# gabraham/flashpca

Measured on AMD Instinct MI355X. Metric: genotype cells/sec (N x P x iters) for k=20 PCA, higher is better.
Workload: dtype i8 (integer genotypes x 7 byte slices of the f64 operand; exact i32 accumulation, f64 recombination; agrees with the f64 kernels to ~3e-15, see fp64_mode); 1 GPU; cfg3: synthetic 500000 samples x 100000 SNPs total, SNP-sharded across GPUs, k=20 (BASELINE configs[2]/[3]); samples=500000, snps_total=100000, snps_per_gpu=100000, k=20, blockvec=16, solver_default_blockvec=16, parallelism=snp-shard x1 + all-reduce(N x b) [single]

## Files before the change

flashpca_amd/_lib.py:

```python
import ctypes as C
import os
import subprocess

HERE = os.path.dirname(os.path.abspath(__file__))
LIB_PATH = os.environ.get("FPCA_LIB") or os.path.join(HERE, "_build", "libfpca.so")
if LIB_PATH == "testhooks":
    LIB_PATH = os.path.join(HERE, "_build", "testhooks", "libfpca.so")
CLI_PATH = os.path.join(HERE, "_build", "flashpca")
HOOKS_LIB_PATH = os.path.join(HERE, "_build", "testhooks", "libfpca.so")
HOOKS_CLI_PATH = os.path.join(HERE, "_build", "testhooks", "flashpca")
CSRC = os.path.join(HERE, "csrc")

STANDARDISE = {"binom": 2, "binom2": 3}
STANDARDISE_DENSE = {"none": 0, "sd": 1, "binom": 2, "binom2": 3, "center": 4}
DIVISOR = {"none": 0, "n1": 1, "p": 2}
UNIQUE_ID_BYTES = 128
SCCA_STATUS = {0: "ok", 1: "maxiter reached", 2: "lambda1 too large", 3: "lambda2 too large"}

ALLREDUCE_FN = C.CFUNCTYPE(C.c_int, C.c_void_p, C.c_void_p, C.c_uint64, C.c_void_p)
COLLECTIVE_FN = C.CFUNCTYPE(C.c_int, C.c_void_p, C.c_void_p, C.c_void_p, C.c_uint64, C.c_void_p)


class PcaOpts(C.Structure):
    _fields_ = [
# ... 120 lines not shown
    "fpca_comm_init_rank": (_I, [_P, _I, _I, _P]),
    "fpca_set_allreduce": (_I, [_P, ALLREDUCE_FN, _P]),
    "fpca_set_collectives": (_I, [_P, COLLECTIVE_FN, COLLECTIVE_FN, _P]),
    "fpca_set_total_snps": (_I, [_P, _U64]),
    "fpca_set_rank": (_I, [_P, _I, _I]),
    "fpca_collective_stats": (_I, [_P, C.POINTER(_U64), C.POINTER(_U64)]),
    "fpca_pca_init_opts": (None, [C.POINTER(PcaOpts), C.c_size_t, C.c_size_t]),
    "fpca_pca_row_ranges": (_I, [_P, C.POINTER(PcaOpts), C.POINTER(_U64), _I]),
    "fpca_pca": (_I, [_P, C.POINTER(PcaOpts), _P, _P, _P, _P, _P, _P, C.POINTER(PcaInfo)]),
    "fpca_check": (_I, [_P, _P, C.c_int64, _P, _I, _I, _P, C.POINTER(_D), C.POINTER(_D)]),
    "fpca_ucca": (_I, [_P, _P, C.c_int64, _I, _I, _P, C.c_int64]),
    "fpca_scca_prepare": (_I, [_P, _P, C.c_int64, _I, _I, _I]),
    "fpca_scca_fit": (_I, [_P, _D, _D, _I, _I, _D, _P, C.c_int64, _P, C.c_int64, _P, C.c_int64, _P, _P, C.c_int64, _P, C.c_int64,
                           C.POINTER(_I), _P, _P, _P, C.POINTER(_I)]),
    "fpca_scca_cv": (_I, [_P, _P, C.c_int64, _I, _P, _I, _P, _I, _P, _I, _I, _I, _I, _I, _D, _P, C.c_int64, C.c_int64, _D, _I, _P, _P, _P, _P, _P, _P,
                          C.POINTER(_D), C.POINTER(_D), C.POINTER(_D), _P, _P]),
    "fpca_bench_apply": (_I, [_P, _I, _I, _I, C.POINTER(BenchResult)]),
    "fpca_profile_begin": (_I, [_P, _I]),
    "fpca_profile_sample_every": (_I, [_P, _I]),
    "fpca_profile_end": (_I, [_P, _I, C.POINTER(BenchResult), C.POINTER(_I)]),
    "fpca_bench_stats": (_I, [_P, _I, C.POINTER(_D), C.POINTER(_D)]),
    "fpca_debug_mfma_probe": (_I, [_P, _P, _P]),
    "fpca_debug_mfma_i8_probe": (_I, [_P, _P, _P]),
    "fpca_debug_mfma_peak": (_I, [_I, _I, _I, C.POINTER(_D)]),
    "fpca_debug_k4": (_I, [_P, _I, _I, _P, _P, _P, _P, _I, _P, _P]),
    "fpca_debug_k4_bench": (_I, [_P, _I, _I, _I, C.POINTER(_D), C.POINTER(_D)]),
    "fpca_debug_k4_fused": (_I, [_P, _I, _I, _P, _P, _P, _P, _P]),
    "fpca_debug_k4_fused_bench": (_I, [_P, _I, _I, _I, C.POINTER(_D)]),
    "fpca_debug_k4_inplace": (_I, [_P, _I, _I, _P, _P, _P, _I, _P, _P]),
    "fpca_debug_fp_plan": (_I, [_P, _I, C.POINTER(_I)]),
    "fpca_debug_poison_partials": (_I, [_P]),
    "fpca_debug_missing_lists": (_I, [_P, _I, _I, _P, _P, _U64, C.POINTER(_U64)]),
    "fpca_debug_gather": (_I, [_I, _I, _P, _P, _U64, _P, _U64, _P, _P, _P, _U64, _U64, _I, _D, _P, C.POINTER(_I)]),
    "fpca_debug_i8_nsc_pad": (_I, [_I, _I, C.POINTER(_I)]),
    "fpca_debug_i8_slices": (_I, [_I, _I, _I, _U64, _U64, _U64, _P, _P, _P, _P, _I, C.POINTER(SlicesOut), C.POINTER(SlicesOut), C.POINTER(_I)]),
    "fpca_debug_i8_instances": (_I, [_P, _I, C.POINTER(_I)]),
    "fpca_debug_gather_blocks": (_I, [_I, _I, _I, _I, _I, _U64, C.POINTER(C.c_uint32), C.POINTER(C.c_uint32), C.POINTER(C.c_uint32)]),
    "fpca_debug_f_sf":(_I, [_D, _U64, _I, C.POINTER(_D), C.POINTER(_D)]),
    "fpca_debug_f_sf_dev": (_I, [_P, _U64, _U64, _I, _P, _P]),
    "fpca_debug_scca_lds": (_I, [_I, C.POINTER(_I), C.POINTER(_I), C.POINTER(_I)]),
    "fpca_debug_fold_stats": (_I, [_P, _P, _I, _P, _I, _P]),
    "fpca_debug_snp_qc_rule": (_I, [_P, _P, _U64, _U64, _D, _D, _P, C.POINTER(_U64)]),
    "fpca_debug_snp_subset_bench": (_I, [_P, _P, _I, C.POINTER(_D), C.POINTER(_D)]),
    "fpca_debug_ld_prune_rule": (_I, [_P, _U64, C.c_uint32, C.c_uint32, _P, _P, _P, _P, C.POINTER(_U64)]),
    "fpca_bench_ld": (_I, [_P, C.c_uint32, _I, _P, C.POINTER(_D)]),
    "fpca_debug_king_rule": (_I, [_P, _P, _U64, _U64, _P, C.POINTER(_U64)]),
# ... 77 lines not shown
```

flashpca_amd/csrc/kernels.hpp:

```cpp
#pragma once
#include <hip/hip_runtime.h>

#include <cstddef>
#include <cstdint>

namespace fpca {
namespace kern {

void repitch(const uint8_t *src, uint64_t np, uint64_t nrec, uint8_t *dst, size_t pitch, hipStream_t stream);
void fix_last_byte(uint8_t *packed, size_t pitch, uint64_t np, int valid_in_last, uint64_t P_g, hipStream_t stream);
void gather_records(const uint8_t *src, size_t pitch, const uint32_t *idx, uint64_t nrec, uint8_t *dst, hipStream_t stream);
void ld_totals(const uint8_t *packed, size_t pitch, uint64_t nrec, uint32_t *tot, hipStream_t stream);
void ld_band(const uint8_t *packed, size_t pitch, const uint32_t *tot, uint32_t npad, uint64_t i0, uint64_t ni, uint64_t jend, uint32_t span,
             double *r2, uint32_t *bits, uint32_t words, double thr, bool force_general, hipStream_t stream);

void bed_stats(const uint8_t *packed, size_t pitch, uint64_t N, uint64_t P_g, int stand_method, double *lut,
               double *mean, double *sd, double *sumsq, uint32_t *nmiss , hipStream_t stream);
void lut_from_meansd(const double *mean, const double *sd, uint64_t P_g, double *lut, hipStream_t stream);

void xt_b(const uint8_t *packed, size_t pitch, const double *lut, const double *B, double *Tpart, uint64_t N_pad,
          uint64_t P_pad, int b, int nsplit, bool fp32, hipStream_t stream);
void x_t(const uint8_t *packed, size_t pitch, const double *lut, const double *T, double *Ypart, uint64_t N_pad,
         uint64_t P_pad, int b, int nsplit, bool fp32, hipStream_t stream);
void reduce_sum(const double *part, double *out, uint64_t count, int nsplit, hipStream_t stream);
// ... 67 lines not shown
   if (!tiled) return (size_t)(r * pitch + q * 16);
   const uint64_t c = q >> 2, kh = (q >> 1) & 1, h = q & 1;
   return (size_t)((r >> 5) * 32 * pitch + c * 2048 + (h * 64 + kh * 32 + (r & 31)) * 16);
}
int gemm_i8_nsc_pad(int S, int b);
size_t gemm_i8_workspace_doubles(uint64_t rows_pad, uint64_t k_pad, int S, int b, bool two);
int gemm_i8_instances(int (*out)[6], int cap);
struct CuFootprint {
   int waves, vgprs, lds_bytes;
};
CuFootprint gemm_i8_footprint(uint64_t rows_pad, int S, int b, bool two, int mode, bool e_only, bool tiled);
void gemm_i8(const uint8_t *packed, size_t pitch, const int8_t *Qg, const int8_t *Qm, const double *wg, const double *wm,
             const long long *colsum_m, const double *mean, const double *sd, double *out, double *ws, uint64_t rows_pad, uint64_t k_pad,
             uint64_t rows_valid, int mode ,
             const double *eplane , int b, int S,
             const SliceOp *next_ops, hipStream_t stream, hipEvent_t *gemm_events = nullptr, hipEvent_t before_combine = nullptr,
             bool e_only = false ,
             bool tiled = false );
void i8_rowscales(const double *mean, const double *sd, uint64_t P_g, uint64_t P_pad, double *inv_sd, double *mu_inv_sd,
                  hipStream_t stream);
void transpose_packed(const uint8_t *in, size_t pitch_in, uint64_t N_pad, uint64_t P_pad, uint8_t *out, size_t pitch_out,
                      hipStream_t stream, bool tiled = false );
void tile_packed(const uint8_t *in, size_t pitch, uint64_t rows, uint8_t *out, hipStream_t stream);
double mfma_i8_peak_tops(int waves_per_simd, int iters, uint32_t fill, hipStream_t stream);
void mfma_i8_probe(const int8_t *A, const int8_t *Bt, int *D, hipStream_t stream);

void gather_packed_rows(const uint8_t *src, size_t pitch, const uint32_t *idx, uint32_t nidx, uint32_t rows_out, uint8_t *dst, hipStream_t stream);
void patch_missing_rows(uint8_t *packed, size_t pitch, const uint32_t *idx, uint32_t nidx, hipStream_t stream);
void scatter_packed_rows(const uint8_t *src, size_t pitch, const uint32_t *idx, uint32_t nidx, uint8_t *packed, hipStream_t stream);
void gather_scaled_rows(const double *V, const double *scale, const uint32_t *idx, uint32_t nidx, uint64_t rows_out, int b, double *dst, hipStream_t stream);
void scatter_rows(const double *src, const uint32_t *idx, uint32_t nidx, int b, double *dst, hipStream_t stream);
void count_missing(const uint8_t *packed, size_t pitch, uint64_t ncols, uint64_t nrec, uint32_t *cnt, hipStream_t stream, bool tiled = false);
void fill_missing(const uint8_t *packed, size_t pitch, uint64_t ncols, uint64_t nrec, const uint32_t *ptr, uint32_t *idx, hipStream_t stream,
                  bool tiled = false);
void sparse_rows_sum(const uint32_t *ptr, const uint32_t *idx, const double *V, const double *rowscale, int b, uint64_t nrec,
                     uint64_t rows_out, double *out, hipStream_t stream, const double *init = nullptr ,
                     bool short_lists = false ,
                     double avg_len = 0 ,
                     unsigned block_limit = 0 );
void sparse_rows_sum_f32(const uint32_t *ptr, const uint32_t *idx, const float *V, const double *colw, int b, uint64_t nrec, uint64_t rows_out,
                         double *out, hipStream_t stream, const double *init = nullptr, bool short_lists = false, double avg_len = 0,
                         unsigned block_limit = 0);
int sparse_rows_sum_variant(int b, bool rowscale, bool short_lists, double avg_len);
unsigned gather_blocks_beside(const CuFootprint &gemm, int gather_vgprs, int ncu);
unsigned sparse_rows_sum_grid(uint64_t rows_out, unsigned block_limit);
unsigned sparse_rows_sum_blocks_beside(const CuFootprint &gemm, int b, bool f32, bool rowscale, bool short_lists, double avg_len);

}
// ... 2 lines not shown
```

flashpca_amd/csrc/kernels_i8.hip:

```cpp
#include <hip/hip_runtime.h>

#include <algorithm>
#include <cmath>
#include <cstdio>
#include <cstdlib>
#include <cstring>
#include <type_traits>
#include <utility>

#include "common.hpp"
#include "dev_scratch.hpp"
#include "kernels.hpp"
#include "launch_check.hpp"

namespace fpca {
namespace kern {

typedef int v4i __attribute__((ext_vector_type(4)));
typedef int v16i __attribute__((ext_vector_type(16)));
typedef double d2 __attribute__((ext_vector_type(2)));
typedef uint32_t u4 __attribute__((ext_vector_type(4)));
typedef uint32_t u2 __attribute__((ext_vector_type(2)));


// ... 520 lines not shown
   const bool idle = C::WAVES == 8 && __builtin_amdgcn_readfirstlane((int)(row0 + (uint64_t)(wr * 32 * MT) >= rows_pad)) != 0;

   v16i acc[MATS][MT][NT];
   v4i acch[MATS][MT][2];
#pragma unroll
   for (int a = 0; a < MATS; a++)
#pragma unroll
      for (int m = 0; m < MT; m++) acch[a][m][0] = acch[a][m][1] = (v4i){0, 0, 0, 0};
#pragma unroll
   for (int a = 0; a < MATS; a++)
#pragma unroll
      for (int m = 0; m < MT; m++)
#pragma unroll
         for (int n = 0; n < NT; n++)
#pragma unroll
            for (int r = 0; r < 16; r++) acc[a][m][n][r] = 0;

   const uint32_t qvoff = (uint32_t)((tid / C::SEGS) * k_pad + (tid % C::SEGS) * 16);
   const uint32_t lds_base = (uint32_t)(size_t)(__attribute__((address_space(3))) unsigned char *)smem;
   const int qdst = (tid / C::SEGS) * LDQ + (tid % C::SEGS) * 16;
   uint32_t pvoff[MT];
#pragma unroll
   for (int m = 0; m < MT; m++)
      pvoff[m] = C::TILED ? (uint32_t)((wr * MT + m) * 32 * pitch + lane * 16)
                          : (uint32_t)((wr * 32 * MT + 32 * m + li) * pitch + kh * (KC / 8));
   const uint8_t *prow = packed + row0 * pitch;
   const uint32_t aQ0 = lds_base + (uint32_t)(wc * 32 * NT + li) * LDQ + kh * (KC / 2);
   const uint32_t aQh0 = lds_base + (uint32_t)(32 * NTF * LDQ + (lane & 15) * C::LDQH) + ((lane >> 5) & 1) * (KC / 2) + ((lane >> 4) & 1) * 16;

   const uint32_t qvoffh = (uint32_t)((tid / 32) * k_pad + (tid % 32) * 8);
   const int qdsth = (tid / 32) * C::LDQH + (tid % 32) * 8;
   u4 qreg[NP];
   u2 qregh[NQ];
   u4 pk[MT][PW], pkn[MT][PW];

   auto issue_q = [&](auto rr, int cc) {
      constexpr int r = decltype(rr)::value, o = r / NP1, r1 = r % NP1;
      const int8_t *sb = ((TWO && o) ? Qm : Qg) + (uint64_t)(col0 + C::RSTEP * r1) * k_pad + (uint64_t)cc * KC;
      if constexpr (C::HALF8 && r1 == NP1 - 1)
         qregh[o] = gload8(sb, qvoffh);
      else
         qreg[r] = gload16<0>(sb, qvoff);
   };
   auto issue_p = [&](u4(&dst)[MT][PW], int cc) {
      const uint8_t *pb = prow + (size_t)cc * (C::TILED ? 2048 : KC / 4);
#pragma unroll
      for (int m = 0; m < MT; m++) {
         dst[m][0] = gload16<0, C::NT_P>(pb, pvoff[m]);
         if constexpr (PW == 2) dst[m][1] = gload16<(C::TILED ? 1024 : 16), C::NT_P>(pb, pvoff[m]);
      }
   };
   auto store_q = [&](auto rr, unsigned char *st, auto behind) {
      constexpr int r = decltype(rr)::value, o = r / NP1, r1 = r % NP1, NB = decltype(behind)::value;
      if constexpr (C::HALF8 && r1 == NP1 - 1) {
         vm_wait<NP - 1 - r + NB>(qregh[o]);
         *reinterpret_cast<u2 *>(st - qdst + qdsth + o * C::QTILE + r1 * C::RSTEP * LDQ) = qregh[o];
      } else {
         vm_wait<NP - 1 - r + NB>(qreg[r]);
         const int hoff = (HALF && r1 == NP1 - 1) ? (tid / C::SEGS) * (C::LDQH - LDQ) : 0;
         *reinterpret_cast<u4 *>(st + o * C::QTILE + r1 * C::RSTEP * LDQ + hoff) = qreg[r];
      }
   };

   constexpr std::integral_constant<int, NPK> after_p{};
   constexpr std::integral_constant<int, 0> after_none{};
   const int c_second = (c_begin + 1 < c_end) ? c_begin + 1 : c_begin;
   if (idle) {
      static_for<NP>([&](auto rr) { issue_q(rr, c_begin); });
      static_for<NP>([&](auto rr) { store_q(rr, smem + qdst, after_none); });
      if constexpr (NBUF == 3) {
         asm volatile("s_waitcnt lgkmcnt(0)" ::: "memory");
         static_for<NP>([&](auto rr) { issue_q(rr, c_second); });
// ... 111 lines not shown
         if constexpr (s == H - 1) issue_p(pkn, cn);
         if constexpr (s >= H) {
            static_for<(s - H + 1) * NP / H - (s - H) * NP / H>([&](auto jj) {
               store_q(std::integral_constant<int, (s - H) * NP / H + decltype(jj)::value>{}, wst, after_p);
            });
         }
         if constexpr (bkey1 != bkey)
            read_b(std::integral_constant<int, ks1>{}, std::integral_constant<int, g1>{}, std::integral_constant<int, (bkey1 & 1)>{}, aQ, aQ2, aQh);
         constexpr bool ahead = NBUF == 3 && last;
         if constexpr (ahead) {
            static_assert(G == 1 && ((NSTEP / MT - 1) & 1) == 1 && ((NSTEP - 1) & AMASK) != 0, "the last micro-step leaves bq[0] and ag[0] free");
#pragma unroll
            for (int mm = 0; mm < MT; mm++)
#pragma unroll
               for (int h = 0; h < PW; h++) {
                  vm_wait<0>(pkn[mm][h]);
                  pk[mm][h] = pkn[mm][h];
               }
            read_b(i0, i0, i0, aQ0 + (uint32_t)bufn * C::STAGE, aQ0 + (uint32_t)bufn * C::STAGE + C::QTILE, aQh0);
         }
         static_for<NG>([&](auto jj) {
            constexpr int j = decltype(jj)::value, n = g * NG + j;
            if constexpr (n < NTF) {
               acc[0][m][n] = __builtin_amdgcn_mfma_i32_32x32x32_i8(ag[akey & AMASK], bq[bkey & 1][0][j], acc[0][m][n], 0, 0, 0);
               if constexpr (MODE == I8_FULL)
                  acc[1][m][n] = __builtin_amdgcn_mfma_i32_32x32x32_i8(am[akey & AMASK], bq[bkey & 1][NQ - 1][j], acc[1][m][n], 0, 0, 0);
            }
            if constexpr (j == 0 && akey1 != akey)
               enz[akey1 & AMASK] = i8_decode<MODE>(pk[m1][ks1 >> 2][ks1 & 3], ag[akey1 & AMASK], am[akey1 & AMASK], tab1);
            if constexpr (j == 0 && ahead) enz[0] = i8_decode<MODE>(pk[0][0][0], ag[0], am[0], tab1);
         });
         if constexpr (HALF && (ks & 1) == 1) {
            v4i t0 = ag[m], t1 = ag[2 + m];
#pragma unroll
            for (int q = 0; q < 4; q++) {
               const auto r = __builtin_amdgcn_permlane16_swap((unsigned)t0[q], (unsigned)t1[q], false, false);
               t0[q] = (int)r[0];
               t1[q] = (int)r[1];
            }
            acch[0][m][0] = __builtin_amdgcn_mfma_i32_16x16x64_i8(t0, bqh, acch[0][m][0], 0, 0, 0);
            acch[0][m][1] = __builtin_amdgcn_mfma_i32_16x16x64_i8(t1, bqh, acch[0][m][1], 0, 0, 0);
            if constexpr (MATS == 2) {
               v4i u0 = am[m], u1 = am[2 + m];
#pragma unroll
               for (int q = 0; q < 4; q++) {
                  const auto r = __builtin_amdgcn_permlane16_swap((unsigned)u0[q], (unsigned)u1[q], false, false);
                  u0[q] = (int)r[0];
                  u1[q] = (int)r[1];
               }
               acch[1][m][0] = __builtin_amdgcn_mfma_i32_16x16x64_i8(u0, TWO ? bqh2 : bqh, acch[1][m][0], 0, 0, 0);
               acch[1][m][1] = __builtin_amdgcn_mfma_i32_16x16x64_i8(u1, TWO ? bqh2 : bqh, acch[1][m][1], 0, 0, 0);
            }
         }
         if constexpr (MODE == I8_SKIP_EMPTY) {
            if (enz[akey & AMASK]) {
               static_for<NG>([&](auto jj) {
                  constexpr int j = decltype(jj)::value, n = g * NG + j;
                  if constexpr (n < NT)
                     acc[1][m][n] = __builtin_amdgcn_mfma_i32_32x32x32_i8(am[akey & AMASK], bq[bkey & 1][NQ - 1][j], acc[1][m][n], 0, 0, 0);
               });
            }
         }
         __builtin_amdgcn_sched_barrier(0);
         if constexpr (bkey1 != bkey) {
            wait_b(std::integral_constant<int, g1>{}, std::integral_constant<int, (bkey1 & 1)>{});
            __builtin_amdgcn_sched_barrier(0);
         }
         if constexpr (ahead) {
            wait_b(i0, i0);
            __builtin_amdgcn_sched_barrier(0);
         }
      });
      if constexpr (NBUF == 3) {
         asm volatile("s_waitcnt lgkmcnt(0)" ::: "memory");
         __builtin_amdgcn_s_barrier();
         asm volatile("" ::: "memory");
         __builtin_amdgcn_sched_barrier(0);
         buf = bufn;
      } else {
#pragma unroll
         for (int m = 0; m < MT; m++)
#pragma unroll
            for (int h = 0; h < PW; h++) {
               vm_wait<0>(pkn[m][h]);
               pk[m][h] = pkn[m][h];
            }
         __syncthreads();
      }
   }

   const int tile0 = (col0 + wc * 32 * NT) / 32;
   double *out = (split == 0 ? part + (((size_t)zblk * rows_pad + row0 + wr * 32 * MT) * 2) * bw
                             : part + (size_t)zb * rows_pad * 2 * bw +
                                  ((((size_t)(split - 1) * zb + zblk) * rowsB + (row0 - rowB0) + wr * 32 * MT) * 2) * bw) +
                 li;
   __syncthreads();
   constexpr int WREG = NT * 4096;
   double *sW = reinterpret_cast<double *>(smem + C::WAVES * WREG);
   constexpr int WCOLS = C::WC * NT * 32;
   for (int t = tid; t < WCOLS; t += C::THREADS) {
      sW[t] = t < C::COLS ? wg[col0 + t] : 0.0;
      sW[WCOLS + t] = t < C::COLS ? wm[col0 + t] : 0.0;
   }
   __syncthreads();
   static_assert(C::LDS_BYTES >= C::WAVES * WREG + 2 * WCOLS * 8, "epilogue LDS layout");
   if (idle) return;
   int *sT = reinterpret_cast<int *>(smem + wave * WREG);
   const double *sWl = sW + wc * 32 * NT + li;
   const int kb = bw / 32;
#pragma unroll
   for (int a = 0; a < MATS; a++)
#pragma unroll
      for (int m = 0; m < MT; m++) {
#pragma unroll
         for (int n = 0; n < NTF; n++) {
            const v16i v = acc[a][m][n];
#pragma unroll
            for (int r = 0; r < 16; r++) sT[(n * 32 + (r & 3) + 8 * (r >> 2) + 4 * kh) * 32 + li] = v[r];
            __builtin_amdgcn_sched_barrier(0);
         }
         if constexpr (HALF) {
#pragma unroll
            for (int t = 0; t < 2; t++)
#pragma unroll
               for (int r = 0; r < 4; r++) {
                  const int row = 16 * t + 4 * (lane >> 4) + r;
                  sT[(NTF * 32 + row) * 32 + (lane & 15)] = acch[a][m][t][r];
                  sT[(NTF * 32 + row) * 32 + 16 + (lane & 15)] = 0;
               }
         }
         __builtin_amdgcn_fence(__ATOMIC_RELEASE, "wavefront");
         __builtin_amdgcn_wave_barrier();
         for (int j = 0; j < 16; j++) {
            const int row = 16 * kh + j;
            for (int k = 0; k < kb; k++) {
               double acc64 = 0.0;
               for (int n = NT - 1 - ((NT - 1 - k) % kb); n >= 0; n -= kb)
                  acc64 += sWl[a * WCOLS + 32 * n] * (double)sT[(n * 32 + row) * 32 + li];
               out[((size_t)(32 * m + row) * 2 + a) * bw + 32 * ((tile0 + k) % kb)] = acc64;
            }
         }
         __builtin_amdgcn_fence(__ATOMIC_ACQUIRE, "wavefront");
         __builtin_amdgcn_wave_barrier();
      }
}

__global__ __launch_bounds__(256) void k_i8_combine(const double *__restrict__ part, int zb, int rows_tile, int nA, int sB, uint64_t rowB0,
                                                     uint64_t rowsB, uint64_t rows_pad, uint64_t rows_valid, int mats,
                                                     const double *__restrict__ eplane ,
                                                     int b, int bw, int S,
                                                     const double *__restrict__ wm, const long long *__restrict__ colsum_m ,
                                                     const double *__restrict__ mean, const double *__restrict__ sd,
                                                     double *__restrict__ out, const double *__restrict__ rs0,
                                                     unsigned long long *__restrict__ bits0, const double *__restrict__ rs1,
                                                     unsigned long long *__restrict__ bits1)
{
   __shared__ double smax[256], sw[9 * 64], sones[64];
   const int c = threadIdx.x % b, r_in = threadIdx.x / b, r_step = 256 / b;
   double m0 = 0.0, m1 = 0.0;
   for (int t = threadIdx.x; t < S * b; t += 256) sw[t] = (mats < 0 || !colsum_m) ? 0.0 : wm[t] * (double)colsum_fold(colsum_m, t);
   __syncthreads();
   if ((int)threadIdx.x < b) {
// ... 445 lines not shown
   if (rows % 256 || pitch % 64) throw Error(-1, "tile_packed: rows in multiples of 256, whole 64-byte chunks per row");
   if (!rows) return;
   hipLaunchKernelGGL(k_tile_packed, dim3((unsigned)(pitch / 64), (unsigned)(rows / 256)), dim3(256), 0, stream, in, pitch, out);
   launch_check();
}

__global__ void k_mfma_i8_probe(const int8_t *A , const int8_t *Bt , int *D)
{
   const int lane = threadIdx.x & 63, li = lane & 31, kh = lane >> 5;
   v4i a = *reinterpret_cast<const v4i *>(A + li * 32 + kh * 16);
   v4i b = *reinterpret_cast<const v4i *>(Bt + li * 32 + kh * 16);
   v16i acc;
   for (int r = 0; r < 16; r++) acc[r] = 0;
   acc = __builtin_amdgcn_mfma_i32_32x32x32_i8(a, b, acc, 0, 0, 0);
   for (int r = 0; r < 16; r++) D[((r & 3) + 8 * (r >> 2) + 4 * kh) * 32 + li] = acc[r];
}

void mfma_i8_probe(const int8_t *A, const int8_t *Bt, int *D, hipStream_t stream)
{
   hipLaunchKernelGGL(k_mfma_i8_probe, dim3(1), dim3(64), 0, stream, A, Bt, D);
   launch_check();
}

__global__ __launch_bounds__(256, 1) void k_mfma_i8_peak(int *out, int iters, uint32_t fill)
{
   const uint32_t l = threadIdx.x * 2654435761u;
   const uint32_t f0 = fill ? (fill ^ l) * 0x9E3779B1u : 0u, f1 = fill ? (f0 >> 3) * 0x85EBCA6Bu : 0u, f2 = fill ? (f1 >> 5) * 0xC2B2AE35u : 0u,
                  f3 = fill ? (f2 >> 7) * 0x27D4EB2Fu : 0u;
   asm volatile(
      "v_mov_b32 v0, 0\n\t"
      "v_mov_b32 v1, 0\n\t"
      "v_mov_b32 v2, 0\n\t"
      "v_mov_b32 v3, 0\n\t"
      "v_mov_b32 v4, 0\n\t"
      "v_mov_b32 v5, 0\n\t"
      "v_mov_b32 v6, 0\n\t"
      "v_mov_b32 v7, 0\n\t"
      "v_mov_b32 v8, 0\n\t"
      "v_mov_b32 v9, 0\n\t"
      "v_mov_b32 v10, 0\n\t"
      "v_mov_b32 v11, 0\n\t"
      "v_mov_b32 v12, 0\n\t"
      "v_mov_b32 v13, 0\n\t"
      "v_mov_b32 v14, 0\n\t"
      "v_mov_b32 v15, 0\n\t"
      "v_mov_b32 v16, 0\n\t"
      "v_mov_b32 v17, 0\n\t"
      "v_mov_b32 v18, 0\n\t"
      "v_mov_b32 v19, 0\n\t"
      "v_mov_b32 v20, 0\n\t"
      "v_mov_b32 v21, 0\n\t"
// ... 83 lines not shown
      "v_mov_b32 v105, 0\n\t"
      "v_mov_b32 v106, 0\n\t"
      "v_mov_b32 v107, 0\n\t"
      "v_mov_b32 v108, 0\n\t"
      "v_mov_b32 v109, 0\n\t"
      "v_mov_b32 v110, 0\n\t"
      "v_mov_b32 v111, 0\n\t"
      "v_mov_b32 v112, 0\n\t"
      "v_mov_b32 v113, 0\n\t"
      "v_mov_b32 v114, 0\n\t"
      "v_mov_b32 v115, 0\n\t"
      "v_mov_b32 v116, 0\n\t"
      "v_mov_b32 v117, 0\n\t"
      "v_mov_b32 v118, 0\n\t"
      "v_mov_b32 v119, 0\n\t"
      "v_mov_b32 v120, 0\n\t"
      "v_mov_b32 v121, 0\n\t"
      "v_mov_b32 v122, 0\n\t"
      "v_mov_b32 v123, 0\n\t"
      "v_mov_b32 v124, 0\n\t"
      "v_mov_b32 v125, 0\n\t"
      "v_mov_b32 v126, 0\n\t"
      "v_mov_b32 v127, 0\n\t"
      ::: "v0", "v1", "v2", "v3", "v4", "v5", "v6", "v7", "v8", "v9", "v10", "v11", "v12", "v13", "v14", "v15", "v16", "v17", "v18", "v19", "v20", "v21", "v22", "v23", "v24", "v25", "v26", "v27", "v28", "v29", "v30", "v31", "v32", "v33", "v34", "v35", "v36", "v37", "v38", "v39", "v40", "v41", "v42", "v43", "v44", "v45", "v46", "v47", "v48", "v49", "v50", "v51", "v52", "v53", "v54", "v55", "v56", "v57", "v58", "v59", "v60", "v61", "v62", "v63", "v64", "v65", "v66", "v67", "v68", "v69", "v70", "v71", "v72", "v73", "v74", "v75", "v76", "v77", "v78", "v79", "v80", "v81", "v82", "v83", "v84", "v85", "v86", "v87", "v88", "v89", "v90", "v91", "v92", "v93", "v94", "v95", "v96", "v97", "v98", "v99", "v100", "v101", "v102", "v103", "v104", "v105", "v106", "v107", "v108", "v109", "v110", "v111", "v112", "v113", "v114", "v115", "v116", "v117", "v118", "v119", "v120", "v121", "v122", "v123", "v124", "v125", "v126", "v127", "v128", "v129", "v130", "v131", "v132", "v133", "v134", "v135", "v136", "v137", "v138", "v139", "v140", "v141", "v142", "v143");
   asm volatile(
      "v_mov_b32 v128, %0\n\t"
      "v_mov_b32 v129, %1\n\t"
      "v_mov_b32 v130, %2\n\t"
      "v_mov_b32 v131, %3\n\t"
      "v_mov_b32 v132, %0\n\t"
      "v_mov_b32 v133, %1\n\t"
      "v_mov_b32 v134, %2\n\t"
      "v_mov_b32 v135, %3\n\t"
      "v_mov_b32 v136, %0\n\t"
      "v_mov_b32 v137, %1\n\t"
      "v_mov_b32 v138, %2\n\t"
      "v_mov_b32 v139, %3\n\t"
      "v_mov_b32 v140, %0\n\t"
      "v_mov_b32 v141, %1\n\t"
      "v_mov_b32 v142, %2\n\t"
      "v_mov_b32 v143, %3\n\t"
      :: "v"(f0), "v"(f1), "v"(f2), "v"(f3) : "v0", "v1", "v2", "v3", "v4", "v5", "v6", "v7", "v8", "v9", "v10", "v11", "v12", "v13", "v14", "v15", "v16", "v17", "v18", "v19", "v20", "v21", "v22", "v23", "v24", "v25", "v26", "v27", "v28", "v29", "v30", "v31", "v32", "v33", "v34", "v35", "v36", "v37", "v38", "v39", "v40", "v41", "v42", "v43", "v44", "v45", "v46", "v47", "v48", "v49", "v50", "v51", "v52", "v53", "v54", "v55", "v56", "v57", "v58", "v59", "v60", "v61", "v62", "v63", "v64", "v65", "v66", "v67", "v68", "v69", "v70", "v71", "v72", "v73", "v74", "v75", "v76", "v77", "v78", "v79", "v80", "v81", "v82", "v83", "v84", "v85", "v86", "v87", "v88", "v89", "v90", "v91", "v92", "v93", "v94", "v95", "v96", "v97", "v98", "v99", "v100", "v101", "v102", "v103", "v104", "v105", "v106", "v107", "v108", "v109", "v110", "v111", "v112", "v113", "v114", "v115", "v116", "v117", "v118", "v119", "v120", "v121", "v122", "v123", "v124", "v125", "v126", "v127", "v128", "v129", "v130", "v131", "v132", "v133", "v134", "v135", "v136", "v137", "v138", "v139", "v140", "v141", "v142", "v143");
   for (int it = 0; it < iters; it++) {
      asm volatile(
         "v_mfma_i32_32x32x32_i8 v[0:15], v[128:131], v[136:139], v[0:15]\n\t"
         "v_mfma_i32_32x32x32_i8 v[16:31], v[132:135], v[136:139], v[16:31]\n\t"
         "v_mfma_i32_32x32x32_i8 v[32:47], v[128:131], v[140:143], v[32:47]\n\t"
         "v_mfma_i32_32x32x32_i8 v[48:63], v[132:135], v[140:143], v[48:63]\n\t"
         "v_mfma_i32_32x32x32_i8 v[64:79], v[128:131], v[136:139], v[64:79]\n\t"
         "v_mfma_i32_32x32x32_i8 v[80:95], v[132:135], v[136:139], v[80:95]\n\t"
         "v_mfma_i32_32x32x32_i8 v[96:111], v[128:131], v[140:143], v[96:111]\n\t"
         "v_mfma_i32_32x32x32_i8 v[112:127], v[132:135], v[140:143], v[112:127]\n\t"
         ::: "v0", "v1", "v2", "v3", "v4", "v5", "v6", "v7", "v8", "v9", "v10", "v11", "v12", "v13", "v14", "v15", "v16", "v17", "v18", "v19", "v20", "v21", "v22", "v23", "v24", "v25", "v26", "v27", "v28", "v29", "v30", "v31", "v32", "v33", "v34", "v35", "v36", "v37", "v38", "v39", "v40", "v41", "v42", "v43", "v44", "v45", "v46", "v47", "v48", "v49", "v50", "v51", "v52", "v53", "v54", "v55", "v56", "v57", "v58", "v59", "v60", "v61", "v62", "v63", "v64", "v65", "v66", "v67", "v68", "v69", "v70", "v71", "v72", "v73", "v74", "v75", "v76", "v77", "v78", "v79", "v80", "v81", "v82", "v83", "v84", "v85", "v86", "v87", "v88", "v89", "v90", "v91", "v92", "v93", "v94", "v95", "v96", "v97", "v98", "v99", "v100", "v101", "v102", "v103", "v104", "v105", "v106", "v107", "v108", "v109", "v110", "v111", "v112", "v113", "v114", "v115", "v116", "v117", "v118", "v119", "v120", "v121", "v122", "v123", "v124", "v125", "v126", "v127", "v128", "v129", "v130", "v131", "v132", "v133", "v134", "v135", "v136", "v137", "v138", "v139", "v140", "v141", "v142", "v143");
   }
   int r;
   asm volatile("s_nop 7\n\ts_nop 7\n\tv_mov_b32 %0, v0" : "=v"(r)::"v0", "v1", "v2", "v3", "v4", "v5", "v6", "v7", "v8", "v9", "v10", "v11", "v12", "v13", "v14", "v15", "v16", "v17", "v18", "v19", "v20", "v21", "v22", "v23", "v24", "v25", "v26", "v27", "v28", "v29", "v30", "v31", "v32", "v33", "v34", "v35", "v36", "v37", "v38", "v39", "v40", "v41", "v42", "v43", "v44", "v45", "v46", "v47", "v48", "v49", "v50", "v51", "v52", "v53", "v54", "v55", "v56", "v57", "v58", "v59", "v60", "v61", "v62", "v63", "v64", "v65", "v66", "v67", "v68", "v69", "v70", "v71", "v72", "v73", "v74", "v75", "v76", "v77", "v78", "v79", "v80", "v81", "v82", "v83", "v84", "v85", "v86", "v87", "v88", "v89", "v90", "v91", "v92", "v93", "v94", "v95", "v96", "v97", "v98", "v99", "v100", "v101", "v102", "v103", "v104", "v105", "v106", "v107", "v108", "v109", "v110", "v111", "v112", "v113", "v114", "v115", "v116", "v117", "v118", "v119", "v120", "v121", "v122", "v123", "v124", "v125", "v126", "v127", "v128", "v129", "v130", "v131", "v132", "v133", "v134", "v135", "v136", "v137", "v138", "v139", "v140", "v141", "v142", "v143");
   if (r == 0x7fffffff) out[threadIdx.x] = r;
}

double mfma_i8_peak_tops(int waves_per_simd, int iters, uint32_t fill, hipStream_t stream)
{
   DevMem<int> d(1024, "fpca_debug_mfma_peak", "the probe's output words");
   const int blocks = 256 * waves_per_simd;
   DevEvent e0("fpca_debug_mfma_peak"), e1("fpca_debug_mfma_peak");
   hipLaunchKernelGGL(k_mfma_i8_peak, dim3(blocks), dim3(256), 0, stream, d.p, iters / 10, fill);
   (void)hipEventRecord(e0, stream);
   hipLaunchKernelGGL(k_mfma_i8_peak, dim3(blocks), dim3(256), 0, stream, d.p, iters, fill);
   (void)hipEventRecord(e1, stream);
   (void)hipEventSynchronize(e1);
   const float ms = elapsed_ms(e0, e1);
   const double ops = (double)blocks * 4  * (double)iters * 8 * 65536.0;
   return ops / (ms * 1e-3) / 1e12;
}

}
}
```

include/fpca_debug.h:

```cpp
#ifndef FPCA_DEBUG_H
#define FPCA_DEBUG_H

#include "fpca.h"

#ifdef __cplusplus
extern "C" {
#endif

typedef struct fpca_bench_result {
   double ms_total;
   double ms_xt;
   double ms_x;
   double ms_allreduce;
   double flops_per_step;
   double packed_bytes_per_step;
   double ms_gemm_xt;
   double ms_gemm_x;
} fpca_bench_result;
int fpca_bench_apply(fpca_ctx *ctx, int b, int steps, int warmup, fpca_bench_result *res);
int fpca_profile_begin(fpca_ctx *ctx, int max_steps);
int fpca_profile_sample_every(fpca_ctx *ctx, int stride);
int fpca_profile_end(fpca_ctx *ctx, int b, fpca_bench_result *res, int *nsteps);
int fpca_bench_stats(fpca_ctx *ctx, int reps, double *ms_per_launch, double *bytes_per_launch);

int fpca_debug_mfma_probe(const double *A, const double *B, double *D);
int fpca_debug_mfma_i8_probe(const int8_t *A, const int8_t *Bt, int32_t *D);
int fpca_debug_mfma_peak(int waves_per_simd, int iters, int pattern, double *tflops);
int fpca_debug_k4(fpca_ctx *ctx, int b, int nq, const double *V, const double *W, double *C_gram, const double *C_in, int use_init,
                  double *Out, double *G_out);
int fpca_debug_k4_fused(fpca_ctx *ctx, int b, int nq, const double *V, const double *W, const double *C_in, double *Out, double *Cg);
int fpca_debug_k4_fused_bench(fpca_ctx *ctx, int b, int nq, int reps, double *ms_fused);
int fpca_debug_k4_inplace(fpca_ctx *ctx, int b, int nq, const double *V, const double *W, const double *C_in, int mode, double *Out,
                          double *G_out);
int fpca_debug_k4_bench(fpca_ctx *ctx, int b, int nq, int reps, double *ms_gram, double *ms_gemm);

int fpca_debug_fp_plan(fpca_ctx *ctx, int b, int out[6]);
int fpca_debug_poison_partials(fpca_ctx *ctx);

int fpca_debug_missing_lists(fpca_ctx *ctx, int b, int by_sample, uint32_t *ptr_out, uint32_t *idx_out, uint64_t idx_cap, uint64_t *nnz);
int fpca_debug_gather(int b, int use_f32, const uint32_t *ptr, const uint32_t *idx, uint64_t nnz, const void *V, uint64_t v_rows,
                      const double *rowscale, const double *colw, const double *init, uint64_t nrec, uint64_t rows_out, int short_lists,
                      double avg_len, double *out, int *variant);

typedef struct fpca_debug_slices_out {
   double *colmax;
   uint64_t *maxbits_own;
   uint64_t *maxbits;
   int8_t *Q;
   int8_t *Qrm;
// ... 42 lines not shown
```

Measured before the change: 80340 billion cells/s.

## Swap MFMA i8 operand order so accumulators hold transposed tiles, vectorise epilogue stores

Exchanges the A and B operands of every i8 MFMA in the gemm kernel so each lane's accumulators hold output columns rather than rows. The epilogue is rewritten to match: LDS staging is transposed, per-lane output pointers change, and results are written as paired double2 stores with two accumulators per loop step. The tiled packed-load offsets are also restructured to share one base offset plus a per-m pointer bump. The likely aim is more contiguous global writes and less per-lane address arithmetic, at the cost of a delicate index remap that must stay exactly consistent with the MFMA output layout. It also adds a debug kernel that checks operand-exchanged MFMA layouts and extends the peak-throughput probe with per-operand fill patterns and a second issue order.

New measurement: 85250 billion cells/s (median of 6 runs). +6.1%, better.

```diff
diff --git a/flashpca_amd/_lib.py b/flashpca_amd/_lib.py
--- a/flashpca_amd/_lib.py
+++ b/flashpca_amd/_lib.py
@@ -166,6 +166,7 @@
     "fpca_bench_stats": (_I, [_P, _I, C.POINTER(_D), C.POINTER(_D)]),
     "fpca_debug_mfma_probe": (_I, [_P, _P, _P]),
     "fpca_debug_mfma_i8_probe": (_I, [_P, _P, _P]),
+    "fpca_debug_mfma_i8_ports": (_I, [_I, _I, _P, _P, _P]),
     "fpca_debug_mfma_peak": (_I, [_I, _I, _I, C.POINTER(_D)]),
     "fpca_debug_k4": (_I, [_P, _I, _I, _P, _P, _P, _P, _I, _P, _P]),
     "fpca_debug_k4_bench": (_I, [_P, _I, _I, _I, C.POINTER(_D), C.POINTER(_D)]),
diff --git a/flashpca_amd/csrc/kernels.hpp b/flashpca_amd/csrc/kernels.hpp
--- a/flashpca_amd/csrc/kernels.hpp
+++ b/flashpca_amd/csrc/kernels.hpp
@@ -113,8 +113,15 @@
 void transpose_packed(const uint8_t *in, size_t pitch_in, uint64_t N_pad, uint64_t P_pad, uint8_t *out, size_t pitch_out,
                       hipStream_t stream, bool tiled = false );
 void tile_packed(const uint8_t *in, size_t pitch, uint64_t rows, uint8_t *out, hipStream_t stream);
-double mfma_i8_peak_tops(int waves_per_simd, int iters, uint32_t fill, hipStream_t stream);
+enum { I8_FILL_ZERO = 0, I8_FILL_RANDOM = 1 , I8_FILL_GENO = 2  };
+struct I8PeakFill {
+   uint32_t seed[4];
+   uint32_t kind[4];
+   int order;
+};
+double mfma_i8_peak_tops(int waves_per_simd, int iters, const I8PeakFill &fill, hipStream_t stream);
 void mfma_i8_probe(const int8_t *A, const int8_t *Bt, int *D, hipStream_t stream);
+void mfma_i8_ports(int shape , bool exchanged, const int8_t *A, const int8_t *Bt, int *D, hipStream_t stream);
 
 void gather_packed_rows(const uint8_t *src, size_t pitch, const uint32_t *idx, uint32_t nidx, uint32_t rows_out, uint8_t *dst, hipStream_t stream);
 void patch_missing_rows(uint8_t *packed, size_t pitch, const uint32_t *idx, uint32_t nidx, hipStream_t stream);
diff --git a/flashpca_amd/csrc/kernels_i8.hip b/flashpca_amd/csrc/kernels_i8.hip
--- a/flashpca_amd/csrc/kernels_i8.hip
+++ b/flashpca_amd/csrc/kernels_i8.hip
@@ -566,7 +566,7 @@
    uint32_t pvoff[MT];
 #pragma unroll
    for (int m = 0; m < MT; m++)
-      pvoff[m] = C::TILED ? (uint32_t)((wr * MT + m) * 32 * pitch + lane * 16)
+      pvoff[m] = C::TILED ? (uint32_t)(wr * MT * 32 * pitch + lane * 16)
                           : (uint32_t)((wr * 32 * MT + 32 * m + li) * pitch + kh * (KC / 8));
    const uint8_t *prow = packed + row0 * pitch;
    const uint32_t aQ0 = lds_base + (uint32_t)(wc * 32 * NT + li) * LDQ + kh * (KC / 2);
@@ -590,8 +590,9 @@
       const uint8_t *pb = prow + (size_t)cc * (C::TILED ? 2048 : KC / 4);
 #pragma unroll
       for (int m = 0; m < MT; m++) {
-         dst[m][0] = gload16<0, C::NT_P>(pb, pvoff[m]);
-         if constexpr (PW == 2) dst[m][1] = gload16<(C::TILED ? 1024 : 16), C::NT_P>(pb, pvoff[m]);
+         const uint8_t *pbm = C::TILED ? pb + (size_t)(32 * m) * pitch : pb;
+         dst[m][0] = gload16<0, C::NT_P>(pbm, pvoff[C::TILED ? 0 : m]);
+         if constexpr (PW == 2) dst[m][1] = gload16<(C::TILED ? 1024 : 16), C::NT_P>(pbm, pvoff[C::TILED ? 0 : m]);
       }
    };
    auto store_q = [&](auto rr, unsigned char *st, auto behind) {
@@ -749,9 +750,9 @@
          static_for<NG>([&](auto jj) {
             constexpr int j = decltype(jj)::value, n = g * NG + j;
             if constexpr (n < NTF) {
-               acc[0][m][n] = __builtin_amdgcn_mfma_i32_32x32x32_i8(ag[akey & AMASK], bq[bkey & 1][0][j], acc[0][m][n], 0, 0, 0);
+               acc[0][m][n] = __builtin_amdgcn_mfma_i32_32x32x32_i8(bq[bkey & 1][0][j], ag[akey & AMASK], acc[0][m][n], 0, 0, 0);
                if constexpr (MODE == I8_FULL)
-                  acc[1][m][n] = __builtin_amdgcn_mfma_i32_32x32x32_i8(am[akey & AMASK], bq[bkey & 1][NQ - 1][j], acc[1][m][n], 0, 0, 0);
+                  acc[1][m][n] = __builtin_amdgcn_mfma_i32_32x32x32_i8(bq[bkey & 1][NQ - 1][j], am[akey & AMASK], acc[1][m][n], 0, 0, 0);
             }
             if constexpr (j == 0 && akey1 != akey)
                enz[akey1 & AMASK] = i8_decode<MODE>(pk[m1][ks1 >> 2][ks1 & 3], ag[akey1 & AMASK], am[akey1 & AMASK], tab1);
@@ -765,8 +766,8 @@
                t0[q] = (int)r[0];
                t1[q] = (int)r[1];
             }
-            acch[0][m][0] = __builtin_amdgcn_mfma_i32_16x16x64_i8(t0, bqh, acch[0][m][0], 0, 0, 0);
-            acch[0][m][1] = __builtin_amdgcn_mfma_i32_16x16x64_i8(t1, bqh, acch[0][m][1], 0, 0, 0);
+            acch[0][m][0] = __builtin_amdgcn_mfma_i32_16x16x64_i8(bqh, t0, acch[0][m][0], 0, 0, 0);
+            acch[0][m][1] = __builtin_amdgcn_mfma_i32_16x16x64_i8(bqh, t1, acch[0][m][1], 0, 0, 0);
             if constexpr (MATS == 2) {
                v4i u0 = am[m], u1 = am[2 + m];
 #pragma unroll
@@ -775,8 +776,8 @@
                   u0[q] = (int)r[0];
                   u1[q] = (int)r[1];
                }
-               acch[1][m][0] = __builtin_amdgcn_mfma_i32_16x16x64_i8(u0, TWO ? bqh2 : bqh, acch[1][m][0], 0, 0, 0);
-               acch[1][m][1] = __builtin_amdgcn_mfma_i32_16x16x64_i8(u1, TWO ? bqh2 : bqh, acch[1][m][1], 0, 0, 0);
+               acch[1][m][0] = __builtin_amdgcn_mfma_i32_16x16x64_i8(TWO ? bqh2 : bqh, u0, acch[1][m][0], 0, 0, 0);
+               acch[1][m][1] = __builtin_amdgcn_mfma_i32_16x16x64_i8(TWO ? bqh2 : bqh, u1, acch[1][m][1], 0, 0, 0);
             }
          }
          if constexpr (MODE == I8_SKIP_EMPTY) {
@@ -784,7 +785,7 @@
                static_for<NG>([&](auto jj) {
                   constexpr int j = decltype(jj)::value, n = g * NG + j;
                   if constexpr (n < NT)
-                     acc[1][m][n] = __builtin_amdgcn_mfma_i32_32x32x32_i8(am[akey & AMASK], bq[bkey & 1][NQ - 1][j], acc[1][m][n], 0, 0, 0);
+                     acc[1][m][n] = __builtin_amdgcn_mfma_i32_32x32x32_i8(bq[bkey & 1][NQ - 1][j], am[akey & AMASK], acc[1][m][n], 0, 0, 0);
                });
             }
          }
@@ -820,7 +821,7 @@
    double *out = (split == 0 ? part + (((size_t)zblk * rows_pad + row0 + wr * 32 * MT) * 2) * bw
                              : part + (size_t)zb * rows_pad * 2 * bw +
                                   ((((size_t)(split - 1) * zb + zblk) * rowsB + (row0 - rowB0) + wr * 32 * MT) * 2) * bw) +
-                 li;
+                 (size_t)li * 2 * bw + 16 * kh;
    __syncthreads();
    constexpr int WREG = NT * 4096;
    double *sW = reinterpret_cast<double *>(smem + C::WAVES * WREG);
@@ -833,7 +834,7 @@
    static_assert(C::LDS_BYTES >= C::WAVES * WREG + 2 * WCOLS * 8, "epilogue LDS layout");
    if (idle) return;
    int *sT = reinterpret_cast<int *>(smem + wave * WREG);
-   const double *sWl = sW + wc * 32 * NT + li;
+   const double *sWl = sW + wc * 32 * NT + 16 * kh;
    const int kb = bw / 32;
 #pragma unroll
    for (int a = 0; a < MATS; a++)
@@ -851,20 +852,22 @@
             for (int t = 0; t < 2; t++)
 #pragma unroll
                for (int r = 0; r < 4; r++) {
-                  const int row = 16 * t + 4 * (lane >> 4) + r;
-                  sT[(NTF * 32 + row) * 32 + (lane & 15)] = acch[a][m][t][r];
-                  sT[(NTF * 32 + row) * 32 + 16 + (lane & 15)] = 0;
+                  const int col = 4 * (lane >> 4) + r;
+                  sT[(NTF * 32 + col) * 32 + 16 * t + (lane & 15)] = acch[a][m][t][r];
+                  sT[(NTF * 32 + 16 + col) * 32 + 16 * t + (lane & 15)] = 0;
                }
          }
          __builtin_amdgcn_fence(__ATOMIC_RELEASE, "wavefront");
          __builtin_amdgcn_wave_barrier();
-         for (int j = 0; j < 16; j++) {
-            const int row = 16 * kh + j;
+         for (int j = 0; j < 16; j += 2) {
+            const int col = 16 * kh + j;
             for (int k = 0; k < kb; k++) {
-               double acc64 = 0.0;
-               for (int n = NT - 1 - ((NT - 1 - k) % kb); n >= 0; n -= kb)
-                  acc64 += sWl[a * WCOLS + 32 * n] * (double)sT[(n * 32 + row) * 32 + li];
-               out[((size_t)(32 * m + row) * 2 + a) * bw + 32 * ((tile0 + k) % kb)] = acc64;
+               double acc0 = 0.0, acc1 = 0.0;
+               for (int n = NT - 1 - ((NT - 1 - k) % kb); n >= 0; n -= kb) {
+                  acc0 += sWl[a * WCOLS + 32 * n + j] * (double)sT[(n * 32 + col) * 32 + li];
+                  acc1 += sWl[a * WCOLS + 32 * n + j + 1] * (double)sT[(n * 32 + col + 1) * 32 + li];
+               }
+               *reinterpret_cast<double2 *>(&out[((size_t)(32 * m) * 2 + a) * bw + 32 * ((tile0 + k) % kb) + j]) = make_double2(acc0, acc1);
             }
          }
          __builtin_amdgcn_fence(__ATOMIC_ACQUIRE, "wavefront");
@@ -1356,11 +1359,52 @@
    launch_check();
 }
 
-__global__ __launch_bounds__(256, 1) void k_mfma_i8_peak(int *out, int iters, uint32_t fill)
+__global__ void k_mfma_i8_ports(int shape, int exchanged, const int8_t *A, const int8_t *Bt, int *D)
+{
+   const int lane = threadIdx.x & 63;
+   if (shape == 32) {
+      const int li = lane & 31, kh = lane >> 5;
+      const v4i a = *reinterpret_cast<const v4i *>(A + li * 32 + kh * 16), b = *reinterpret_cast<const v4i *>(Bt + li * 32 + kh * 16);
+      v16i acc;
+      for (int r = 0; r < 16; r++) acc[r] = 0;
+      acc = exchanged ? __builtin_amdgcn_mfma_i32_32x32x32_i8(b, a, acc, 0, 0, 0) : __builtin_amdgcn_mfma_i32_32x32x32_i8(a, b, acc, 0, 0, 0);
+      for (int r = 0; r < 16; r++) D[((r & 3) + 8 * (r >> 2) + 4 * kh) * 32 + li] = acc[r];
+   } else {
+      const int lj = lane & 15, qd = lane >> 4;
+      const v4i a = *reinterpret_cast<const v4i *>(A + lj * 64 + qd * 16), b = *reinterpret_cast<const v4i *>(Bt + lj * 64 + qd * 16);
+      v4i acc = {0, 0, 0, 0};
+      acc = exchanged ? __builtin_amdgcn_mfma_i32_16x16x64_i8(b, a, acc, 0, 0, 0) : __builtin_amdgcn_mfma_i32_16x16x64_i8(a, b, acc, 0, 0, 0);
+      for (int r = 0; r < 4; r++) D[(4 * qd + r) * 16 + lj] = acc[r];
+   }
+}
+
+void mfma_i8_ports(int shape, bool exchanged, const int8_t *A, const int8_t *Bt, int *D, hipStream_t stream)
+{
+   hipLaunchKernelGGL(k_mfma_i8_ports, dim3(1), dim3(64), 0, stream, shape, exchanged ? 1 : 0, A, Bt, D);
+   launch_check();
+}
+
+#define I8_PEAK_CLOBBERS "v0", "v1", "v2", "v3", "v4", "v5", "v6", "v7", "v8", "v9", "v10", "v11", "v12", "v13", "v14", "v15", "v16", "v17", "v18", "v19", "v20", "v21", "v22", "v23", "v24", "v25", "v26", "v27", "v28", "v29", "v30", "v31", "v32", "v33", "v34", "v35", "v36", "v37", "v38", "v39", "v40", "v41", "v42", "v43", "v44", "v45", "v46", "v47", "v48", "v49", "v50", "v51", "v52", "v53", "v54", "v55", "v56", "v57", "v58", "v59", "v60", "v61", "v62", "v63", "v64", "v65", "v66", "v67", "v68", "v69", "v70", "v71", "v72", "v73", "v74", "v75", "v76", "v77", "v78", "v79", "v80", "v81", "v82", "v83", "v84", "v85", "v86", "v87", "v88", "v89", "v90", "v91", "v92", "v93", "v94", "v95", "v96", "v97", "v98", "v99", "v100", "v101", "v102", "v103", "v104", "v105", "v106", "v107", "v108", "v109", "v110", "v111", "v112", "v113", "v114", "v115", "v116", "v117", "v118", "v119", "v120", "v121", "v122", "v123", "v124", "v125", "v126", "v127", "v128", "v129", "v130", "v131", "v132", "v133", "v134", "v135", "v136", "v137", "v138", "v139", "v140", "v141", "v142", "v143"
+__global__ __launch_bounds__(256, 1) void k_mfma_i8_peak(int *out, int iters, I8PeakFill fl)
 {
    const uint32_t l = threadIdx.x * 2654435761u;
-   const uint32_t f0 = fill ? (fill ^ l) * 0x9E3779B1u : 0u, f1 = fill ? (f0 >> 3) * 0x85EBCA6Bu : 0u, f2 = fill ? (f1 >> 5) * 0xC2B2AE35u : 0u,
-                  f3 = fill ? (f2 >> 7) * 0x27D4EB2Fu : 0u;
+   uint32_t f[4][4];
+#pragma unroll
+   for (int s = 0; s < 4; s++) {
+      const uint32_t kind = fl.kind[s];
+      uint32_t h[4];
+      h[0] = (fl.seed[s] ^ l) * 0x9E3779B1u;
+      h[1] = (h[0] >> 3) * 0x85EBCA6Bu;
+      h[2] = (h[1] >> 5) * 0xC2B2AE35u;
+      h[3] = (h[2] >> 7) * 0x27D4EB2Fu;
+#pragma unroll
+      for (int q = 0; q < 4; q++) {
+         uint32_t g = 0;
+#pragma unroll
+         for (int k = 0; k < 4; k++) g |= ((((h[q] >> (8 * k)) & 0xffu) * 3u) >> 8) << (8 * k);
+         f[s][q] = kind == I8_FILL_ZERO ? 0u : kind == I8_FILL_GENO ? g : h[q];
+      }
+   }
    asm volatile(
       "v_mov_b32 v0, 0\n\t"
       "v_mov_b32 v1, 0\n\t"
@@ -1490,43 +1534,58 @@
       "v_mov_b32 v125, 0\n\t"
       "v_mov_b32 v126, 0\n\t"
       "v_mov_b32 v127, 0\n\t"
-      ::: "v0", "v1", "v2", "v3", "v4", "v5", "v6", "v7", "v8", "v9", "v10", "v11", "v12", "v13", "v14", "v15", "v16", "v17", "v18", "v19", "v20", "v21", "v22", "v23", "v24", "v25", "v26", "v27", "v28", "v29", "v30", "v31", "v32", "v33", "v34", "v35", "v36", "v37", "v38", "v39", "v40", "v41", "v42", "v43", "v44", "v45", "v46", "v47", "v48", "v49", "v50", "v51", "v52", "v53", "v54", "v55", "v56", "v57", "v58", "v59", "v60", "v61", "v62", "v63", "v64", "v65", "v66", "v67", "v68", "v69", "v70", "v71", "v72", "v73", "v74", "v75", "v76", "v77", "v78", "v79", "v80", "v81", "v82", "v83", "v84", "v85", "v86", "v87", "v88", "v89", "v90", "v91", "v92", "v93", "v94", "v95", "v96", "v97", "v98", "v99", "v100", "v101", "v102", "v103", "v104", "v105", "v106", "v107", "v108", "v109", "v110", "v111", "v112", "v113", "v114", "v115", "v116", "v117", "v118", "v119", "v120", "v121", "v122", "v123", "v124", "v125", "v126", "v127", "v128", "v129", "v130", "v131", "v132", "v133", "v134", "v135", "v136", "v137", "v138", "v139", "v140", "v141", "v142", "v143");
+      ::: I8_PEAK_CLOBBERS);
    asm volatile(
       "v_mov_b32 v128, %0\n\t"
       "v_mov_b32 v129, %1\n\t"
       "v_mov_b32 v130, %2\n\t"
       "v_mov_b32 v131, %3\n\t"
-      "v_mov_b32 v132, %0\n\t"
-      "v_mov_b32 v133, %1\n\t"
-      "v_mov_b32 v134, %2\n\t"
-      "v_mov_b32 v135, %3\n\t"
-      "v_mov_b32 v136, %0\n\t"
-      "v_mov_b32 v137, %1\n\t"
-      "v_mov_b32 v138, %2\n\t"
-      "v_mov_b32 v139, %3\n\t"
-      "v_mov_b32 v140, %0\n\t"
-      "v_mov_b32 v141, %1\n\t"
-      "v_mov_b32 v142, %2\n\t"
-      "v_mov_b32 v143, %3\n\t"
-      :: "v"(f0), "v"(f1), "v"(f2), "v"(f3) : "v0", "v1", "v2", "v3", "v4", "v5", "v6", "v7", "v8", "v9", "v10", "v11", "v12", "v13", "v14", "v15", "v16", "v17", "v18", "v19", "v20", "v21", "v22", "v23", "v24", "v25", "v26", "v27", "v28", "v29", "v30", "v31", "v32", "v33", "v34", "v35", "v36", "v37", "v38", "v39", "v40", "v41", "v42", "v43", "v44", "v45", "v46", "v47", "v48", "v49", "v50", "v51", "v52", "v53", "v54", "v55", "v56", "v57", "v58", "v59", "v60", "v61", "v62", "v63", "v64", "v65", "v66", "v67", "v68", "v69", "v70", "v71", "v72", "v73", "v74", "v75", "v76", "v77", "v78", "v79", "v80", "v81", "v82", "v83", "v84", "v85", "v86", "v87", "v88", "v89", "v90", "v91", "v92", "v93", "v94", "v95", "v96", "v97", "v98", "v99", "v100", "v101", "v102", "v103", "v104", "v105", "v106", "v107", "v108", "v109", "v110", "v111", "v112", "v113", "v114", "v115", "v116", "v117", "v118", "v119", "v120", "v121", "v122", "v123", "v124", "v125", "v126", "v127", "v128", "v129", "v130", "v131", "v132", "v133", "v134", "v135", "v136", "v137", "v138", "v139", "v140", "v141", "v142", "v143");
-   for (int it = 0; it < iters; it++) {
-      asm volatile(
-         "v_mfma_i32_32x32x32_i8 v[0:15], v[128:131], v[136:139], v[0:15]\n\t"
-         "v_mfma_i32_32x32x32_i8 v[16:31], v[132:135], v[136:139], v[16:31]\n\t"
-         "v_mfma_i32_32x32x32_i8 v[32:47], v[128:131], v[140:143], v[32:47]\n\t"
-         "v_mfma_i32_32x32x32_i8 v[48:63], v[132:135], v[140:143], v[48:63]\n\t"
-         "v_mfma_i32_32x32x32_i8 v[64:79], v[128:131], v[136:139], v[64:79]\n\t"
-         "v_mfma_i32_32x32x32_i8 v[80:95], v[132:135], v[136:139], v[80:95]\n\t"
-         "v_mfma_i32_32x32x32_i8 v[96:111], v[128:131], v[140:143], v[96:111]\n\t"
-         "v_mfma_i32_32x32x32_i8 v[112:127], v[132:135], v[140:143], v[112:127]\n\t"
-         ::: "v0", "v1", "v2", "v3", "v4", "v5", "v6", "v7", "v8", "v9", "v10", "v11", "v12", "v13", "v14", "v15", "v16", "v17", "v18", "v19", "v20", "v21", "v22", "v23", "v24", "v25", "v26", "v27", "v28", "v29", "v30", "v31", "v32", "v33", "v34", "v35", "v36", "v37", "v38", "v39", "v40", "v41", "v42", "v43", "v44", "v45", "v46", "v47", "v48", "v49", "v50", "v51", "v52", "v53", "v54", "v55", "v56", "v57", "v58", "v59", "v60", "v61", "v62", "v63", "v64", "v65", "v66", "v67", "v68", "v69", "v70", "v71", "v72", "v73", "v74", "v75", "v76", "v77", "v78", "v79", "v80", "v81", "v82", "v83", "v84", "v85", "v86", "v87", "v88", "v89", "v90", "v91", "v92", "v93", "v94", "v95", "v96", "v97", "v98", "v99", "v100", "v101", "v102", "v103", "v104", "v105", "v106", "v107", "v108", "v109", "v110", "v111", "v112", "v113", "v114", "v115", "v116", "v117", "v118", "v119", "v120", "v121", "v122", "v123", "v124", "v125", "v126", "v127", "v128", "v129", "v130", "v131", "v132", "v133", "v134", "v135", "v136", "v137", "v138", "v139", "v140", "v141", "v142", "v143");
-   }
+      "v_mov_b32 v132, %4\n\t"
+      "v_mov_b32 v133, %5\n\t"
+      "v_mov_b32 v134, %6\n\t"
+      "v_mov_b32 v135, %7\n\t"
+      "v_mov_b32 v136, %8\n\t"
+      "v_mov_b32 v137, %9\n\t"
+      "v_mov_b32 v138, %10\n\t"
+      "v_mov_b32 v139, %11\n\t"
+      "v_mov_b32 v140, %12\n\t"
+      "v_mov_b32 v141, %13\n\t"
+      "v_mov_b32 v142, %14\n\t"
+      "v_mov_b32 v143, %15\n\t"
+      :: "v"(f[0][0]), "v"(f[0][1]), "v"(f[0][2]), "v"(f[0][3]), "v"(f[1][0]), "v"(f[1][1]), "v"(f[1][2]), "v"(f[1][3]), "v"(f[2][0]), "v"(f[2][1]), "v"(f[2][2]), "v"(f[2][3]), "v"(f[3][0]), "v"(f[3][1]), "v"(f[3][2]), "v"(f[3][3]) : I8_PEAK_CLOBBERS);
+   if (fl.order == 0)
+      for (int it = 0; it < iters; it++) {
+         asm volatile(
+            "v_mfma_i32_32x32x32_i8 v[0:15], v[128:131], v[136:139], v[0:15]\n\t"
+            "v_mfma_i32_32x32x32_i8 v[16:31], v[132:135], v[136:139], v[16:31]\n\t"
+            "v_mfma_i32_32x32x32_i8 v[32:47], v[128:131], v[140:143], v[32:47]\n\t"
+            "v_mfma_i32_32x32x32_i8 v[48:63], v[132:135], v[140:143], v[48:63]\n\t"
+            "v_mfma_i32_32x32x32_i8 v[64:79], v[128:131], v[136:139], v[64:79]\n\t"
+            "v_mfma_i32_32x32x32_i8 v[80:95], v[132:135], v[136:139], v[80:95]\n\t"
+            "v_mfma_i32_32x32x32_i8 v[96:111], v[128:131], v[140:143], v[96:111]\n\t"
+            "v_mfma_i32_32x32x32_i8 v[112:127], v[132:135], v[140:143], v[112:127]\n\t"
+            ::: I8_PEAK_CLOBBERS);
+      }
+   else
+      for (int it = 0; it < iters; it++) {
+         asm volatile(
+            "v_mfma_i32_32x32x32_i8 v[0:15], v[128:131], v[136:139], v[0:15]\n\t"
+            "v_mfma_i32_32x32x32_i8 v[16:31], v[128:131], v[140:143], v[16:31]\n\t"
+            "v_mfma_i32_32x32x32_i8 v[32:47], v[132:135], v[136:139], v[32:47]\n\t"
+            "v_mfma_i32_32x32x32_i8 v[48:63], v[132:135], v[140:143], v[48:63]\n\t"
+            "v_mfma_i32_32x32x32_i8 v[64:79], v[128:131], v[136:139], v[64:79]\n\t"
+            "v_mfma_i32_32x32x32_i8 v[80:95], v[128:131], v[140:143], v[80:95]\n\t"
+            "v_mfma_i32_32x32x32_i8 v[96:111], v[132:135], v[136:139], v[96:111]\n\t"
+            "v_mfma_i32_32x32x32_i8 v[112:127], v[132:135], v[140:143], v[112:127]\n\t"
+            ::: I8_PEAK_CLOBBERS);
+      }
    int r;
-   asm volatile("s_nop 7\n\ts_nop 7\n\tv_mov_b32 %0, v0" : "=v"(r)::"v0", "v1", "v2", "v3", "v4", "v5", "v6", "v7", "v8", "v9", "v10", "v11", "v12", "v13", "v14", "v15", "v16", "v17", "v18", "v19", "v20", "v21", "v22", "v23", "v24", "v25", "v26", "v27", "v28", "v29", "v30", "v31", "v32", "v33", "v34", "v35", "v36", "v37", "v38", "v39", "v40", "v41", "v42", "v43", "v44", "v45", "v46", "v47", "v48", "v49", "v50", "v51", "v52", "v53", "v54", "v55", "v56", "v57", "v58", "v59", "v60", "v61", "v62", "v63", "v64", "v65", "v66", "v67", "v68", "v69", "v70", "v71", "v72", "v73", "v74", "v75", "v76", "v77", "v78", "v79", "v80", "v81", "v82", "v83", "v84", "v85", "v86", "v87", "v88", "v89", "v90", "v91", "v92", "v93", "v94", "v95", "v96", "v97", "v98", "v99", "v100", "v101", "v102", "v103", "v104", "v105", "v106", "v107", "v108", "v109", "v110", "v111", "v112", "v113", "v114", "v115", "v116", "v117", "v118", "v119", "v120", "v121", "v122", "v123", "v124", "v125", "v126", "v127", "v128", "v129", "v130", "v131", "v132", "v133", "v134", "v135", "v136", "v137", "v138", "v139", "v140", "v141", "v142", "v143");
+   asm volatile("s_nop 7\n\ts_nop 7\n\tv_mov_b32 %0, v0" : "=v"(r)::I8_PEAK_CLOBBERS);
    if (r == 0x7fffffff) out[threadIdx.x] = r;
 }
-
-double mfma_i8_peak_tops(int waves_per_simd, int iters, uint32_t fill, hipStream_t stream)
+#undef I8_PEAK_CLOBBERS
+
+double mfma_i8_peak_tops(int waves_per_simd, int iters, const I8PeakFill &fill, hipStream_t stream)
 {
    DevMem<int> d(1024, "fpca_debug_mfma_peak", "the probe's output words");
    const int blocks = 256 * waves_per_simd;
diff --git a/include/fpca_debug.h b/include/fpca_debug.h
--- a/include/fpca_debug.h
+++ b/include/fpca_debug.h
@@ -25,6 +25,7 @@
 
 int fpca_debug_mfma_probe(const double *A, const double *B, double *D);
 int fpca_debug_mfma_i8_probe(const int8_t *A, const int8_t *Bt, int32_t *D);
+int fpca_debug_mfma_i8_ports(int shape, int exchanged, const int8_t *A, const int8_t *Bt, int32_t *D);
 int fpca_debug_mfma_peak(int waves_per_simd, int iters, int pattern, double *tflops);
 int fpca_debug_k4(fpca_ctx *ctx, int b, int nq, const double *V, const double *W, double *C_gram, const double *C_in, int use_init,
                   double *Out, double *G_out);
```
